# ztaylor797/APMBackend

Measured on AMD Instinct MI355X. Metric: log-lines/sec z-scored (whole node), higher is better.
Workload: dtype fp64

## Files before the change

apmbackend_amd/csrc/bindings.cpp:

```cpp
#include <pybind11/pybind11.h>
#include <pybind11/stl.h>

#include <cstring>
#include <memory>

#include "kernels/kernel_api.h"
#include "runtime/engine.h"
#include "runtime/format.h"
#include "runtime/jsutil.h"
#include "runtime/merge.h"

namespace apm {
namespace copyenc {
void encode_blob(std::string_view blob, std::string* out, int64_t* counts);
}
int apm_txcopy_lines(const char* d_text, const uint64_t* h_line_off, int64_t n, std::string& out_rows);
std::vector<double> apm_release_bench(int64_t n, int iters, uint64_t seed);
}

namespace py = pybind11;
using namespace apm;

void register_tailer(py::module_& m);
void register_synth(py::module_& m);
// ... 324 lines not shown
        py::gil_scoped_release rel;
        return c.all_reduce_host(v, max);
      }, py::arg("values"), py::arg("max") = false)
      .def("all_gather", [](Collective& c, py::bytes b) {
        std::string s = b;
        std::vector<uint8_t> v(s.begin(), s.end()), out;
        { py::gil_scoped_release rel; out = c.all_gather_host(v); }
        return py::bytes((const char*)out.data(), out.size());
      })
      .def("abort", &Collective::abort)
      .def("aborted", &Collective::aborted)
      .def_property_readonly("rank", &Collective::rank)
      .def_property_readonly("nranks", &Collective::nranks);
  py::class_<LocalGroup, std::shared_ptr<LocalGroup>>(m, "LocalCollGroup")
      .def(py::init([](int n, double timeout_ms) { return make_local_group(n, timeout_ms); }), py::arg("n"),
           py::arg("timeout_ms") = 120000.0);

  py::class_<Engine>(m, "Engine")
      .def(py::init([](const py::dict& d) { return new Engine(config_from(d)); }))
      .def("add_file", &Engine::add_file)
      .def("add_server", &Engine::add_server)
      .def("set_override", [](Engine& e, const std::string& svc, const py::dict& d) { e.set_override(svc, override_from(d)); })
      .def("clear_overrides", &Engine::clear_overrides)
      .def("refresh_series_settings", &Engine::refresh_series_settings)
      .def("stage_reconfig", [](Engine& e, const py::dict& ecfg, const py::dict& overrides, uint64_t gen) {
        const EngineConfig c = config_from(ecfg);
        ReconfigSpec r;
        r.gen = gen;
        r.n_lags = c.n_lags;
        for (int l = 0; l < MAX_LAGS; ++l) {
          r.lags[l] = c.lags[l]; r.thr[l] = c.thr[l]; r.infl[l] = c.infl[l]; r.lag_suppressed[l] = c.lag_suppressed[l];
        }
        r.alert_window = c.alert_window; r.alert_threshold = c.alert_threshold; r.both_only = c.both_only;
        r.hard_min_ms = c.hard_min_ms; r.hard_min_tpm = c.hard_min_tpm; r.hard_max_ms = c.hard_max_ms;
        r.cooldown_ms = c.cooldown_ms;
        r.interval_len = c.interval_len; r.window = c.window; r.buffer = c.buffer;
        for (auto kv : overrides) r.overrides[kv.first.cast<std::string>()] = override_from(kv.second.cast<py::dict>());
        e.stage_reconfig(r);
      }, py::arg("ecfg"), py::arg("overrides"), py::arg("gen"))
      .def("reconfig_info", [](Engine& e) {
        py::dict d;
        d["applied_gen"] = e.reconfig_applied_gen(); d["applied"] = e.reconfigs_applied();
        d["lag_set_changes"] = e.lag_set_changes();
        d["window_changes"] = e.window_changes();
        d["ring_slots"] = e.ring_slots();
        d["ring_grows"] = e.ring_grows();
        return d;
      })
      .def("lag_values", &Engine::lag_values)
      .def("cache_stats", [](Engine& e, bool drain) {
        std::vector<uint64_t> v;
        { py::gil_scoped_release rel; v = e.cache_stats(drain); }
        py::dict d;
        if (v.size() == 6) {
          d["slots"] = v[0]; d["occupied"] = v[1]; d["acct"] = v[2]; d["record"] = v[3]; d["partials"] = v[4];
          d["need"] = v[5];
        }
        return d;
      }, py::arg("drain") = true)
      .def("process_batch",
           [](Engine& e, py::buffer buf, const std::vector<std::tuple<int32_t, uint64_t, uint64_t>>& chunks,
              double now) {
             py::buffer_info bi = buf.request();
             const uint8_t* p = (const uint8_t*)bi.ptr;
             const uint64_t n = (uint64_t)(bi.size * bi.itemsize);
             auto ch = chunks_from(chunks);
             py::gil_scoped_release rel;
             e.process_batch(p, n, ch, now);
           },
           py::arg("buf"), py::arg("chunks"), py::arg("now") = -1.0)
      .def("process_batch_ptr",
           [](Engine& e, uintptr_t ptr, uint64_t n, const std::vector<std::tuple<int32_t, uint64_t, uint64_t>>& chunks,
              double now, uintptr_t next_ptr, uint64_t next_n,
              const std::vector<std::tuple<int32_t, uint64_t, uint64_t>>& next_chunks) {
             auto ch = chunks_from(chunks);
             auto nch = chunks_from(next_chunks);
             py::gil_scoped_release rel;
             e.process_batch((const uint8_t*)ptr, n, ch, now, next_ptr ? (const uint8_t*)next_ptr : nullptr, next_n,
                             next_ptr ? &nch : nullptr);
           },
           py::arg("ptr"), py::arg("n"), py::arg("chunks"), py::arg("now") = -1.0, py::arg("next_ptr") = 0,
           py::arg("next_n") = 0,
           py::arg("next_chunks") = std::vector<std::tuple<int32_t, uint64_t, uint64_t>>())
      .def("stage_batch_ptr",
           [](Engine& e, uintptr_t ptr, uint64_t n) {
             py::gil_scoped_release rel;
             e.stage_batch((const uint8_t*)ptr, n);
           },
           py::arg("ptr"), py::arg("n"))
      .def("process_tx_lines", [](Engine& e, py::bytes b, double now) {
             std::string v = b;
             py::gil_scoped_release rel;
             e.process_tx_lines(v, now);
           }, py::arg("blob"), py::arg("now") = -1.0)
      .def("take", &Engine::take, py::call_guard<py::gil_scoped_release>())
      .def("flush", &Engine::flush, py::call_guard<py::gil_scoped_release>())
      .def("dump_state", [](Engine& e, const std::string& path, const std::string& reason) {
        py::gil_scoped_release rel;
        return e.dump_state(path, reason);
      })
      .def("save_state", [](Engine& e, const std::string& path, py::bytes extra) {
             std::string x = extra;
             py::gil_scoped_release rel;
             return e.save_state(path, x);
           }, py::arg("path"), py::arg("extra") = py::bytes(""))
      .def("checkpoint_async", [](Engine& e, const std::string& prefix, py::bytes extra, bool force_base) {
             std::string x = extra;
             py::gil_scoped_release rel;
             return e.checkpoint_async(prefix, x, force_base);
           }, py::arg("prefix"), py::arg("extra") = py::bytes(""), py::arg("force_base") = false)
      .def("checkpoint_wait", &Engine::checkpoint_wait, py::call_guard<py::gil_scoped_release>())
      .def("checkpoint_info", [](Engine& e) {
        const CheckpointInfo c = e.checkpoint_info();
        py::dict d;
        d["busy"] = c.busy; d["done"] = c.done; d["skipped"] = c.skipped; d["sync_fallbacks"] = c.sync_fallbacks;
        d["chain_len"] = c.chain_len; d["last_base"] = c.last_base; d["last_stall_ms"] = c.last_stall_ms;
        d["last_write_ms"] = c.last_write_ms; d["last_bytes"] = c.last_bytes; d["stage_bytes"] = c.stage_bytes;
        d["last_deferred_bytes"] = c.last_deferred_bytes;
        d["streamed"] = c.streamed; d["streamed_live_rows"] = c.streamed_live_rows;
        d["side_rows"] = c.side_rows; d["guard_stalls"] = c.guard_stalls; d["stage_cap"] = c.stage_cap;
        d["last_ring_rows"] = c.last_ring_rows;
        return d;
      })
      .def("export_series", &Engine::export_series, py::call_guard<py::gil_scoped_release>())
      .def("import_series", &Engine::import_series, py::call_guard<py::gil_scoped_release>())
      .def("export_buckets", [](Engine& e) {
        BucketDump d;
        { py::gil_scoped_release rel; d = e.export_buckets(); }
        return py::make_tuple(d.latest, d.series, d.bucket, d.count, d.values);
      })
      .def("import_buckets", &Engine::import_buckets, py::call_guard<py::gil_scoped_release>())
      .def("export_history", [](Engine& e, int lag_idx, int32_t lo, int32_t hi) {
        std::vector<int32_t> len;
        std::vector<double> vals;
        { py::gil_scoped_release rel; e.export_history(lag_idx, lo, hi, len, vals); }
        return py::make_tuple(len, py::bytes((const char*)vals.data(), vals.size() * 8));
      })
      .def("import_history", [](Engine& e, int lag_idx, const std::vector<int32_t>& series,
                                const std::vector<int32_t>& len, py::bytes vals) {
        std::string b = vals;
        std::vector<double> v(b.size() / 8);
        std::memcpy(v.data(), b.data(), v.size() * 8);
        py::gil_scoped_release rel;
        e.import_history(lag_idx, series, len, v);
      })
      .def("export_lag_settings", &Engine::export_lag_settings)
      .def("export_pending", &Engine::export_pending, py::call_guard<py::gil_scoped_release>())
      .def("import_pending", &Engine::import_pending, py::call_guard<py::gil_scoped_release>())
      .def("export_cooldowns", &Engine::export_cooldowns)
      .def("import_cooldowns", &Engine::import_cooldowns)
      .def("export_alert_counters", &Engine::export_alert_counters)
      .def("import_alert_counters", &Engine::import_alert_counters)
      .def("cooldown_by_service", &Engine::cooldown_by_service)
      .def("set_trace", &Engine::set_trace)
      .def("take_trace", [](Engine& e) {
        std::vector<TraceEvent> t;
        { py::gil_scoped_release rel; t = e.take_trace(); }
        py::list out;
        for (auto& x : t) out.append(py::make_tuple(std::string(x.name), x.t0_ms, x.t1_ms, x.tid, x.batch));
        return out;
      })
      .def("set_server_context", &Engine::set_server_context, py::arg("server"), py::arg("ts_ms"),
           py::arg("gauges"), py::arg("host_load") = 0.0)
      .def("load_state", [](Engine& e, const std::string& path) {
             std::string x;
             { py::gil_scoped_release rel; x = e.load_state(path); }
// ... 418 lines not shown
```

apmbackend_amd/csrc/runtime/devjoin.h:

```cpp
#pragma once
#include <hip/hip_runtime.h>

#include <atomic>
#include <cstdint>
#include <deque>
#include <functional>
#include <mutex>
#include <string>
#include <unordered_map>
#include <vector>

#include "../apm_types.h"
#include "../kernels/devjoin_api.h"
#include "hipres.h"
#include "join.h"

namespace apm {

struct CopySegs;

struct DevJoinConfig {
  uint32_t max_events = 1u << 20;
  uint64_t max_batch_bytes = 64ull << 20;
  uint32_t max_chunks = 4096;
  int table_bits = 21;
  int reg_bits = 20;
  uint32_t max_raw = 1u << 20;
  uint32_t arena_cap = 1u << 20;
  uint32_t pool_blocks = 0;
  uint64_t ring_bytes = 4ull << 30;
  double record_ttl_ms = 120000, acct_ttl_ms = 120000, need_ttl_ms = 30000;
  TzTable tz{};
  int device = 0;
};

struct DevJoinBatch {
  int slot = 0;
  uint32_t n_out = 0, n_stats = 0, n_db = 0, n_dropped = 0;
  std::vector<std::pair<uint32_t, int64_t>> cands;
  std::vector<std::pair<uint32_t, int32_t>> unresolved;
  std::string text_tx, text_db;
  uint64_t ring_base = 0;
  int64_t max_bucket = INT64_MIN;
  TxRec* d_tx = nullptr;
  int32_t* d_raw = nullptr;
  int64_t* d_gid = nullptr;
};

class DeviceJoin {
 public:
  DeviceJoin(const DevJoinConfig& cfg, Dictionary* dict, const std::vector<FileInfo>* files,
             const std::vector<std::string>* servers);
  ~DeviceJoin();

  uint8_t* d_bytes(int k) { return sl_[k].d_bytes; }
  uint8_t* d_stage() {
    if (!d_stage_bytes_) {
      d_stage_bytes_ = (uint8_t*)res_.dmalloc_on(stream_, cfg_.max_batch_bytes + 256);
      HIP_OK(hipStreamSynchronize(stream_));
    }
    return d_stage_bytes_;
  }
  void swap_stage(int k) { std::swap(sl_[k].d_bytes, d_stage_bytes_); }
  Event* d_events(int k) { return sl_[k].d_events; }
  void select_host(int k, const uint32_t* d_n_ev, uint32_t max_ev, hipStream_t ps);
  void set_chunks(int k, const std::vector<int32_t>& chunk_file, const uint32_t* d_chunk_file,
                  const uint8_t* d_chunk_kind);
  void chunk_upload(int k, uint32_t max_ev, CopySegs& cs);
  void export_select(int k, CopySegs& cs);
  using ParallelFor = std::function<void(int, const std::function<void(int)>&)>;
  void run(int k, const uint8_t* host_bytes, uint32_t n_ev, uint64_t n_bytes, double now, uint64_t batch_no, bool want_tx,
           bool want_db, DevJoinBatch& out, const ParallelFor& parallel = nullptr,
           const std::function<void()>* meanwhile = nullptr);
  void prepass_ahead(int k, const uint8_t* host_bytes, const ParallelFor& parallel);
  void release_slot(int k, hipStream_t stats_stream);

  int32_t raw_server(int32_t raw) const { return raw_info_[raw].server; }
  int32_t raw_service(int32_t raw) const { return raw_info_[raw].norm_id; }
  int32_t n_raw() const { return n_raw_.load(std::memory_order_acquire); }
  int32_t* d_raw_series() { return d_raw_series_; }

  char* ring() { return d_ring_; }
  uint64_t ring_cap() const { return cfg_.ring_bytes; }
  void set_ring_low(uint64_t low);
  uint64_t ring_head() const { return ring_head_.load(std::memory_order_acquire); }
  uint64_t ring_low() const { return ring_low_.load(std::memory_order_acquire); }
  uint64_t keys_live() const { return keys_live_ + keys_since_rebuild_; }
  uint64_t need_live() const { return arena_head_ - (regions_.empty() ? arena_head_ : regions_.front().lo); }
  uint64_t ring_reserve(uint64_t bytes);
  void reset_ring(uint64_t head);

  JoinCounters counters() const;
  std::vector<uint64_t> cache_stats(double now, bool sync = true);

  void save(class BinWriter& w);
  void load(class BinReader& r);
  static constexpr int kPhases = 8;
  double phase_t[kPhases + 1] = {0};
  std::vector<std::pair<const char*, std::pair<double, double>>> spans;
  std::vector<std::pair<const char*, std::pair<double, double>>> save_spans;
  const JoinCounts& last_counts() const { return *h_counts_; }
  size_t device_bytes() const { return res_.device_bytes(); }
  size_t trim(double now);

 private:
  struct Slot {
    uint8_t* d_bytes = nullptr;
    Event* d_events = nullptr;
    uint8_t* host_flag = nullptr;
    uint32_t* d_mh_idx = nullptr;
    uint32_t* d_walk_idx = nullptr;
    AudF* d_aud = nullptr;
    SelCount* d_n_host = nullptr;
    Mapped<Event> h_host_ev;
    Mapped<uint32_t> h_host_idx;
    Mapped<SelCount> h_n_host;
    int32_t* d_chunk_next = nullptr;
    uint8_t* d_chunk_first = nullptr;
    Mapped<int32_t> h_chunk_next;
    Mapped<uint8_t> h_chunk_first;
    const uint32_t* d_chunk_file = nullptr;
    const uint8_t* d_chunk_kind = nullptr;
    uint32_t n_chunks = 0;
    std::vector<int32_t> chunk_file;
    TxRec* d_tx = nullptr;
    int32_t* d_tx_raw = nullptr;
    int64_t* d_tx_gid = nullptr;
    hipEvent_t free_ev = nullptr;
    bool used = false;
  } sl_[2];

  struct RawInfo { int32_t server; int32_t norm_id; uint64_t svc; };

  struct PrepassTask {
    int32_t file = -1;
    std::vector<uint32_t> idx;
    std::vector<HostOp> hops;
    std::string hbuf;
    uint64_t audit_errors = 0, invalid_acct = 0, pm_host = 0;
    uint32_t put(std::string_view s) { const uint32_t o = (uint32_t)hbuf.size(); hbuf.append(s.data(), s.size()); return o; }
  };
  void host_prepass(int k, const uint8_t* host_bytes, uint32_t n_host, const ParallelFor& parallel,
                    std::vector<HostOp>& hops, std::string& hbuf);
  void host_event(PrepassTask& t, const Event& e, uint32_t ev, const uint8_t* host_bytes);
  void on_app(PrepassTask& t, const Event& e, uint32_t ev, std::string_view line);
  void save_tables(class BinWriter& w);
  void aud_reserve(AudGen& g, uint32_t autr, uint32_t items, uint64_t txt);
// ... 12 lines not shown
  void grow_pool(uint64_t need_free);
  uint64_t pool_avail(bool exact);
  void ensure_tmp();

  DevJoinConfig cfg_;
  uint32_t init_table_cap_ = 0, init_arena_cap_ = 0;
  Dictionary* dict_;
  const std::vector<FileInfo>* files_;
  const std::vector<std::string>* servers_;
  hipStream_t stream_ = nullptr;
  HipRes res_;
  uint8_t* d_stage_bytes_ = nullptr;

  std::vector<HostOp> hops_;
  std::string hbuf_;
  std::vector<HostOp> hops_ahead_;
  std::string hbuf_ahead_;
  int ahead_k_ = -1;
  PinnedBuf<HostOp> h_hops_;
  PinnedBuf<uint8_t> h_hbuf_;
  HostOp* d_hops_ = nullptr;
  uint8_t* d_hbuf_ = nullptr;
  size_t d_hops_cap_ = 0, d_hbuf_cap_ = 0;
  std::vector<PrepassTask> tasks_;
  void* d_sel_tmp_ = nullptr;
  size_t sel_tmp_bytes_ = 0;
  uint64_t audit_errors_ = 0, host_pm_ = 0, host_invalid_acct_ = 0, host_events_ = 0, events_ = 0, tx_ = 0, tx_db_ = 0;

  DJArgs a_{};
  DJFormatArgs f_{};
  KeyState* d_table_ = nullptr;
  uint64_t* d_keys_ = nullptr;
  uint32_t keys_cap_ = 0;
  bool keys_stale_ = true;
  void sync_keys();
  unsigned long long* d_cstats_ = nullptr;
  unsigned long long* h_cstats_ = nullptr;
  unsigned long long cstats_last_[5] = {0, 0, 0, 0, 0};
  uint32_t cstats_cap_ = 0, cstats_last_cap_ = 0;
  hipEvent_t cstats_ev_ = nullptr;
  bool cstats_pending_ = false, cstats_have_ = false;
  KeyState* d_table_spare_ = nullptr;
  uint32_t table_cap_ = 0;
  uint64_t keys_since_rebuild_ = 0, keys_live_ = 0;
  bool live_pending_ = false;
  hipEvent_t live_ev_ = nullptr;
  uint32_t* d_rb_scratch_ = nullptr;
  size_t rb_scratch_bytes_ = 0;
  uint8_t* d_pool_ = nullptr;
  uint32_t* d_pool_ring_ = nullptr;
  uint32_t pool_n_ = 0;
  unsigned long long* h_live_ = nullptr;
  uint64_t table_grows_ = 0, arena_grows_ = 0, pool_grows_ = 0, table_rebuilds_ = 0, trims_ = 0;
  RegSlot* d_reg_ = nullptr;
  RegMiss* d_miss_ = nullptr;
  RegMiss* h_miss_ = nullptr;
  uint32_t miss_cap_ = 0;
  NeedEnt* d_arena_ = nullptr;
  uint64_t arena_head_ = 0;
  struct Region { uint64_t lo, hi; double exp; };
  std::deque<Region> regions_;
  uint64_t* d_exp_lo_ = nullptr;
  uint64_t* d_exp_hi_ = nullptr;
  Mapped<uint64_t> h_exp_;
  SoapState* d_soap_ = nullptr;
  AudGen aud_gen_[2]{};
  int aud_cur_ = 0;
  uint64_t* d_sel_val_ = nullptr;
  uint64_t* d_sel_pos_ = nullptr;
  uint64_t *d_aud_key_ = nullptr, *d_aud_key_sorted_ = nullptr;
  uint32_t *d_aud_ord_ = nullptr, *d_aud_ord_sorted_ = nullptr;
  uint32_t aud_key_cap_ = 0;
  uint32_t* d_walk_lo_ = nullptr;
  int32_t* d_file_first_ = nullptr;
  AudItem* d_aud_slots_ = nullptr;
  uint32_t aud_slots_cap_ = 0;
  static constexpr size_t kCkBounce = 32u << 20;
  char* h_ck_bounce_ = nullptr;
  uint32_t soap_cap_ = 0;
  int32_t* d_file_server_ = nullptr;
  uint64_t* d_file_skey_ = nullptr;
  uint64_t* d_file_fkey_ = nullptr;
  std::vector<uint64_t> h_file_skey_, h_file_fkey_;
  void sync_file_keys();
  size_t files_uploaded_ = 0;
  RawSvc* d_rawtab_ = nullptr;
  int32_t* d_raw_series_ = nullptr;
  int32_t* d_raw_first_ = nullptr;
  std::vector<RawInfo> raw_info_;
  std::atomic<int32_t> n_raw_{0};
  std::string names_;
  std::unordered_map<std::string, int32_t> name_off_;
  char* d_names_ = nullptr;
  size_t names_uploaded_ = 0, names_cap_ = 0;
  int32_t* d_reg_fill_ = nullptr;
  int32_t* h_reg_fill_ = nullptr;
  RawSvc* h_rawtab_ = nullptr;
  TxDev* d_out_ = nullptr;
  uint32_t out_cap_ = 0;
  uint32_t* d_lens_ = nullptr;
  uint32_t* d_offs_ = nullptr;
  int64_t* d_bucket_ = nullptr;
  int64_t* d_bmax_ = nullptr;
  uint32_t* d_cand_ = nullptr;
  int64_t* d_cand_bucket_ = nullptr;
  uint32_t* d_unres_ = nullptr;
  uint32_t* h_cand_ = nullptr;
  int64_t* h_cand_bucket_ = nullptr;
  uint32_t* h_unres_ = nullptr;
  char* d_txt_tx_ = nullptr;
  char* d_txt_db_ = nullptr;
  size_t txt_cap_ = 0;
  PinnedBuf<char> h_txt_;
  uint32_t last_tx_bytes_ = 0, last_db_bytes_ = 0, last_cands_ = 0;
  uint64_t* d_ring_pos_ = nullptr;
  uint32_t* d_slot_head_ = nullptr;
  uint32_t heads_cap_ = 0;
  uint32_t* d_big_ = nullptr;
  uint64_t write_regrows_ = 0;
  void ensure_txt(size_t bytes);
  void* d_tmp_ = nullptr;
  size_t tmp_bytes_ = 0;
  JoinCounts* d_counts_ = nullptr;
  JoinCounts* h_counts_ = nullptr;
  unsigned long long* d_live_ = nullptr;
  JOp* d_ops_ = nullptr;
  uint8_t* d_soap_code_ = nullptr;
  double* d_soap_num_ = nullptr;
  uint64_t* d_soap_hash_ = nullptr;
  uint32_t* d_chunk_ev_lo_ = nullptr;
  uint32_t* d_seg_f_ = nullptr;
  uint32_t* d_seg_in_ = nullptr;
  uint64_t* d_chain_hash_ = nullptr;
  uint32_t *d_op_slot_ = nullptr, *d_op_slot_sorted_ = nullptr, *d_op_idx_ = nullptr, *d_op_idx_sorted_ = nullptr;
  uint64_t *d_exp_key_ = nullptr, *d_exp_key_sorted_ = nullptr;
  uint32_t *d_exp_idx_ = nullptr, *d_exp_idx_sorted_ = nullptr, *d_exp_cnt_ = nullptr, *d_exp_pos_ = nullptr;
  uint32_t exp_cap_ = 0;
  uint32_t* d_out_cnt_ = nullptr;
  uint32_t* d_out_pos_ = nullptr;
  TxDev* d_stage_ = nullptr;
  DJOverflow* d_ovf_ = nullptr;
  char* d_ring_ = nullptr;
  std::mutex ring_mu_;
  std::atomic<uint64_t> ring_head_{0};
  std::atomic<uint64_t> ring_low_{0};
};

}
```

apmbackend_amd/csrc/runtime/engine.cpp:

```cpp
#include <cstdlib>
#include "engine.h"

#include <pthread.h>
#include <sched.h>

#include <cctype>
#include <fstream>

#include <rocprofiler-sdk-roctx/roctx.h>

#include <unistd.h>

#include <cerrno>
#include <cstring>

#include <algorithm>
#include <exception>
#include <chrono>
#include <cmath>
#include <cstring>
#include <queue>
#include <stdexcept>

#include "../kernels/devjoin_api.h"
// ... 663 lines not shown

void Engine::refresh_series_settings() {
  flush();
  for (int l = 0; l < MAX_LAGS; ++l) { alias_thr_[l] = cfg_.thr[l]; alias_infl_[l] = cfg_.infl[l]; }
  std::vector<int32_t> order(n_series_);
  for (int32_t i = 0; i < n_series_; ++i) order[i] = i;
  std::sort(order.begin(), order.end(), [&](int32_t a, int32_t b) { return series_[a].emit_key < series_[b].emit_key; });
  for (int32_t s : order) if (zscore_seen_[s]) apply_series_settings(s);
  upload_series_tables(0);
}

void Engine::upload_series_tables(int32_t lo) {
  const int32_t n = n_series_;
  if (lo < 0) lo = 0;
  if (n <= lo) return;
  const size_t m = (size_t)(n - lo);
  const int L = cfg_.n_lags;
  char* st = stage(m * (8 * (2 * L + 2) + 1));
  double* col = (double*)st;
  for (int l = 0; l < L; ++l) {
    double* t = col + (size_t)(2 * l) * m;
    double* f = col + (size_t)(2 * l + 1) * m;
    for (size_t i = 0; i < m; ++i) {
      t[i] = h_thr_[(size_t)(lo + i) * MAX_LAGS + l];
      f[i] = h_infl_[(size_t)(lo + i) * MAX_LAGS + l];
    }
    h2d(lag_[l].thr + lo, t, m * 8, stream_);
    h2d(lag_[l].infl + lo, f, m * 8, stream_);
  }
  double* hm = col + (size_t)(2 * L) * m;
  uint64_t* ek = (uint64_t*)(col + (size_t)(2 * L + 1) * m);
  uint8_t* sp = (uint8_t*)(col + (size_t)(2 * L + 2) * m);
  std::memcpy(hm, h_hard_max_.data() + lo, m * 8);
  std::memcpy(ek, h_emit_key_.data() + lo, m * 8);
  std::memcpy(sp, h_suppressed_.data() + lo, m);
  h2d(d_hard_max_ + lo, hm, m * 8, stream_);
  h2d(d_emit_key_ + lo, ek, m * 8, stream_);
  h2d(d_suppressed_ + lo, sp, m, stream_);
  stage_done();
  if (want(OUT_SL)) upload_slo_classes(lo);
}

void Engine::upload_slo_classes(int32_t lo) {
  const int32_t n = n_series_;
  lo = std::min(lo, slo_cls_uploaded_);
  if (lo == 0 || h_slo_cls_.size() != (size_t)n) {
    h_slo_cls_.resize((size_t)n);
    for (int32_t s = 0; s < n; ++s) h_slo_cls_[s] = slo_class_of(s);
    lo = 0;
  }
  if (n > lo) {
    const size_t mc = (size_t)(n - lo);
    int32_t* cs = (int32_t*)stage(mc * 4);
    std::memcpy(cs, h_slo_cls_.data() + lo, mc * 4);
    h2d(d_slo_cls_ + lo, cs, mc * 4, stream_);
    stage_done();
  }
  slo_cls_uploaded_ = n;
}

std::vector<uint64_t> Engine::cache_stats(bool drain) {
  if (drain) flush();
  if (dj_) {
    if (drain) HIP_OK(hipStreamSynchronize(parse_stream_));
    return dj_->cache_stats(watermark_, drain);
  }
  return {};
}

JoinCounters Engine::join_counters() const {
  if (dj_) return dj_->counters();
  JoinCounters t;
  for (auto& s : shards_) {
    const JoinCounters& c = s->counters;
    t.events += c.events; t.tx += c.tx; t.tx_db += c.tx_db; t.expired_partials += c.expired_partials;
    t.need_expired += c.need_expired; t.ejb_exit_unmatched += c.ejb_exit_unmatched;
    t.invalid_acct += c.invalid_acct; t.audit_errors += c.audit_errors; t.host_fallback += c.host_fallback;
  }
  return t;
}

void Engine::launch_parse(ParseSlot& ps, const uint8_t* host_bytes, uint64_t n_bytes, const std::vector<Chunk>& chunks_in,
                          bool speculative) {
  const double t0 = now_ms();
  if (n_bytes > cfg_.max_batch_bytes) throw std::runtime_error("batch larger than max_batch_bytes");
  if (chunks_in.size() > cfg_.max_chunks) throw std::runtime_error("too many chunks in batch");
  std::vector<size_t> order(chunks_in.size());
  for (size_t i = 0; i < order.size(); ++i) order[i] = i;
  std::stable_sort(order.begin(), order.end(), [&](size_t a, size_t b) {
    return files_[chunks_in[a].file].server < files_[chunks_in[b].file].server;
  });
  ps.chunk_file.assign(chunks_in.size(), 0);
  uint64_t off = 0;
  bool canonical = true;
  for (size_t k = 0; k < order.size(); ++k) {
    const Chunk& c = chunks_in[k];
    if (order[k] != k || c.begin != off) { canonical = false; break; }
    off = c.end;
  }
  canonical = canonical && off == n_bytes && n_bytes + 64 <= cfg_.max_batch_bytes + 256;
  ps.hb = ps.h_bytes;
  if (canonical) {
    ps.hb = host_bytes;
    for (size_t k = 0; k < order.size(); ++k) {
      const Chunk& c = chunks_in[k];
      if (c.end > c.begin && host_bytes[c.end - 1] != '\n') throw std::runtime_error("chunk must end with a newline");
      ps.h_chunk_begin[k] = (uint32_t)c.begin;
      ps.h_chunk_kind[k] = files_[c.file].kind;
      ps.h_chunk_file[k] = (uint32_t)c.file;
      ps.chunk_file[k] = c.file;
    }
  } else {
    off = 0;
    const bool in_place = host_bytes == ps.h_bytes;
    std::vector<uint8_t> tmp_copy;
    const uint8_t* src = host_bytes;
    if (in_place) {
      tmp_copy.assign(host_bytes, host_bytes + n_bytes);
      src = tmp_copy.data();
    }
    for (size_t k = 0; k < order.size(); ++k) {
      const Chunk& c = chunks_in[order[k]];
      const uint64_t len = c.end - c.begin;
      if (len > 0 && src[c.end - 1] != '\n') throw std::runtime_error("chunk must end with a newline");
      std::memcpy(ps.h_bytes + off, src + c.begin, len);
      ps.h_chunk_begin[k] = (uint32_t)off;
      ps.h_chunk_kind[k] = files_[c.file].kind;
      ps.h_chunk_file[k] = (uint32_t)c.file;
      ps.chunk_file[k] = c.file;
      off += len;
    }
    std::memset(ps.h_bytes + off, 0, 64);
  }
  const uint32_t n_chunks = (uint32_t)order.size();
  ps.h_chunk_begin[n_chunks] = (uint32_t)off;
  ps.n_bytes = off;
  ps.src = host_bytes;
  ps.src_n = n_bytes;
  metrics_.bytes += off;
  ++metrics_.batches;

  const int k = (int)(&ps - pslot_);
  bool staged = false;
  if (dev() && canonical && in_stage_src_ == host_bytes && in_stage_n_ == n_bytes && in_stage_ev_) {
    HIP_OK(hipStreamWaitEvent(parse_stream_, in_stage_ev_, 0));
    dj_->swap_stage(k);
    staged = true;
    ++metrics_.staged_batches;
  }
  in_stage_src_ = nullptr;
  in_stage_n_ = 0;
  uint8_t* dbytes = dev() ? dj_->d_bytes(k) : d_bytes_;
  Event* devents = dev() ? dj_->d_events(k) : d_events_;
  if (!staged) HIP_OK(hipMemcpyAsync(dbytes, ps.hb, off, hipMemcpyHostToDevice, parse_stream_));
  {
    CopySegs up;
    up.add(d_chunk_begin_[k], HipRes::device_alias(ps.h_chunk_begin), (size_t)(n_chunks + 1) * 4);
    up.add(d_chunk_kind_[k], HipRes::device_alias(ps.h_chunk_kind), n_chunks + 1);
    up.add(d_chunk_file_[k], HipRes::device_alias(ps.h_chunk_file), (size_t)(n_chunks + 1) * 4);
    if (dev()) {
      dj_->set_chunks(k, ps.chunk_file, d_chunk_file_[k], d_chunk_kind_[k]);
      dj_->chunk_upload(k, cfg_.max_lines, up);
    }
    apm_copy_segs(&up, parse_stream_);
  }
  if (apm_parse_batch(dbytes, off, d_chunk_begin_[k], d_chunk_kind_[k], d_chunk_file_[k], n_chunks, d_parse_ws_,
                      cfg_.max_lines, devents, d_counts_, d_counts_ + 1, d_watermark_, d_file_open_, &cfg_.tz,
                      parse_stream_) != 0)
    throw std::runtime_error("parse workspace too small");
  if (dev()) dj_->select_host(k, d_counts_, cfg_.max_lines, parse_stream_);
  {
    CopySegs ex;
    ex.add(HipRes::device_alias(ps.h_counts), d_counts_, 8);
    ex.add(HipRes::device_alias(ps.h_watermark), d_watermark_, 8);
    if (dev()) dj_->export_select(k, ex);
    apm_copy_segs(&ex, parse_stream_);
  }
  ps.spec_copied = 0;
  if (speculative && !dev() && spec_events_) {
    ps.spec_copied = std::min<uint32_t>(spec_events_, cfg_.max_lines);
    HIP_OK(hipMemcpyAsync(ps.h_events, d_events_, (size_t)ps.spec_copied * sizeof(Event), hipMemcpyDeviceToHost,
                          parse_stream_));
  }
  ps.pending = true;
  metrics_.t_parse_ms += now_ms() - t0;
}

void Engine::stage_batch(const uint8_t* host_bytes, uint64_t n_bytes) {
  if (!dev() || !host_bytes || n_bytes == 0 || n_bytes > cfg_.max_batch_bytes) return;
  const double t0 = now_ms();
  if (!in_stage_stream_) {
    HIP_OK(hipStreamCreateWithFlags(&in_stage_stream_, hipStreamNonBlocking));
    res_.adopt(in_stage_stream_);
    in_stage_ev_ = res_.new_event();
  }
  HIP_OK(hipMemcpyAsync(dj_->d_stage(), host_bytes, n_bytes, hipMemcpyHostToDevice, in_stage_stream_));
  HIP_OK(hipEventRecord(in_stage_ev_, in_stage_stream_));
  in_stage_src_ = host_bytes;
  in_stage_n_ = n_bytes;
  trace_event("stage H2D (launch)", t0, now_ms(), 0);
}

void Engine::finish_parse(ParseSlot& ps) {
  const double t0 = now_ms();
  HIP_OK(hipStreamSynchronize(parse_stream_));
  ps.n_events = ps.h_counts[0];
  ps.n_lines = ps.h_counts[1];
  if (ps.n_lines > cfg_.max_lines) throw std::runtime_error("batch has more lines than max_lines");
  metrics_.lines += ps.n_lines;
  metrics_.events += ps.n_events;
  if (!dev() && ps.n_events > ps.spec_copied) {
    const uint32_t lo = ps.spec_copied;
    HIP_OK(hipMemcpyAsync(ps.h_events + lo, d_events_ + lo, (size_t)(ps.n_events - lo) * sizeof(Event),
                          hipMemcpyDeviceToHost, parse_stream_));
    HIP_OK(hipStreamSynchronize(parse_stream_));
  }
  ps.spec_copied = 0;
  spec_events_ = ps.n_events + ps.n_events / 4 + 1024;
  ps.pending = false;
  last_slot_ = (int)(&ps - pslot_);
  metrics_.t_parse_ms += now_ms() - t0;
}

static void merge_shard_outputs(const std::vector<std::vector<TxOut>>& outs, bool multi, std::vector<TxOut>& txs) {
  txs.clear();
  const int ns = (int)outs.size();
  size_t total = 0;
  std::vector<size_t> split(ns, 0);
  for (int k = 0; k < ns; ++k) {
    auto& v = outs[k];
    total += v.size();
    size_t p = 0;
    while (p < v.size() && !(v[p].seq >> 63)) ++p;
    split[k] = p;
  }
  txs.reserve(total);
  using Item = std::pair<uint64_t, std::pair<int, size_t>>;
  std::priority_queue<Item, std::vector<Item>, std::greater<Item>> pq;
  for (int k = 0; k < ns; ++k)
    if (split[k] > 0) pq.push({outs[k][0].seq, {k, 0}});
  while (!pq.empty()) {
    auto it = pq.top();
    pq.pop();
    auto& v = outs[it.second.first];
    txs.push_back(v[it.second.second]);
    const size_t nx = it.second.second + 1;
// ... 63 lines not shown
    };
    const uint32_t nc = (uint32_t)chunk_file.size();
    uint32_t c = 0;
    while (c < nc) {
      const int32_t srv = files_[chunk_file[c]].server;
      uint32_t d = c + 1;
      while (d < nc && files_[chunk_file[d]].server == srv) ++d;
      const uint32_t lo = first_event_of_chunk(c), hi = first_event_of_chunk(d);
      if (hi > lo) shard_range[srv].push_back({lo, hi});
      c = d;
    }
  }
  shard_ms_.assign(shards_.size() * 16, 0.0);
  shard_maxb_.assign(shards_.size() * 8, INT64_MIN);
  pool_->run((int)shards_.size(), [&](int s) {
    const double ts0 = now_ms();
    JoinShard& sh = *shards_[s];
    sh.out().clear();
    sh.begin_batch(clock, batch_no_);
    for (const auto& r : shard_range[s]) sh.process(h_events + r.first, r.second - r.first, hb, chunk_file);
    if (lockstep_) {
      int64_t b = INT64_MIN;
      for (const TxOut& t : sh.out()) {
        if (t.to_db || !(t.end_ms == t.end_ms) || t.end_ms < 10000) continue;
        const int64_t tb = (int64_t)t.end_ms / 10000;
        if (tb > b) b = tb;
      }
      shard_maxb_[(size_t)s * 8] = b;
    }
    const double ts1 = now_ms();
    shard_ms_[(size_t)s * 16] = ts1 - ts0;
    trace_event("shard", ts0, ts1, 2 + s);
  }, launch_next ? &launch_next_parse : nullptr);
  const double t1b = now_ms();
  metrics_.t_join_shards_ms += t1b - t1;
  {
    double sum = 0, mx = 0;
    for (size_t s = 0; s < shards_.size(); ++s) { sum += shard_ms_[s * 16]; mx = std::max(mx, shard_ms_[s * 16]); }
    metrics_.t_shard_busy_ms += shards_.empty() ? 0 : sum / shards_.size();
    metrics_.t_shard_max_ms += mx;
  }
  std::vector<std::vector<TxOut>> outs(shards_.size());
  {
    std::lock_guard<std::mutex> g(out_pool_mu_);
    for (size_t k = 0; k < shards_.size(); ++k) {
      outs[k].swap(shards_[k]->out());
      if (!out_pool_.empty()) {
        shards_[k]->out().swap(out_pool_.back());
        out_pool_.pop_back();
      }
    }
  }
  bool multi = false;
  for (auto& r : shard_range) multi |= r.size() > 1;
  const double t2 = now_ms();
  metrics_.t_join_ms += t2 - t1;
  metrics_.t_merge_ms += t2 - t1b;
  roctxRangePop();
  trace_event("join", t1, t1b, 0);
  trace_event("handoff", t1b, t2, 0);

  int sync_slot = -1;
  if (lockstep_) {
    int64_t bmax = INT64_MIN;
    for (size_t k = 0; k < shards_.size(); ++k) bmax = std::max(bmax, shard_maxb_[k * 8]);
    sync_slot = lockstep_collect(bmax);
  } else {
    watermark_ = batch_watermark(ps);
  }

  const double tp0 = now_ms();
  post_stats(std::move(outs), multi, t0, sync_slot);
  const double tp1 = now_ms();
  trace_event("post", tp0, tp1, 0);
  if (coll_) fleet_exchange_upto(fleet_posted_ - 1);
  trace_event("fleet.exchange", tp1, now_ms(), 0);
  metrics_.t_total_ms += now_ms() - t0;
  ++batch_no_;
}

void Engine::process_batch_dev_tail(ParseSlot& ps, double t0, double now_override, const uint8_t* next_bytes,
                                    uint64_t next_n, const std::vector<Chunk>* next_chunks) {
  const int k = (int)(&ps - pslot_);
  if (next_bytes && next_chunks) {
    launch_parse(pslot_[k ^ 1], next_bytes, next_n, *next_chunks, true);
    prefetched_ = true;
  }
  cur_slot_ = k ^ 1;
  last_n_events_ = ps.n_events;
  const double t1 = now_ms();
  roctxRangePop();
  roctxRangePushA("apm.join");
  trace_event("parse", t0, t1, 0);
  const double clock = now_override >= 0 ? now_override : watermark_;
  if (lockstep_) lockstep_issue(batch_watermark(ps));
  DevJoinBatch b;
  const DeviceJoin::ParallelFor par = [this](int n, const std::function<void(int)>& fn) { pool_->run(n, fn); };
  const std::function<void()> ahead = [this, k, par]() {
    if (!ahead_lane_) ahead_lane_.reset(new TaskLane());
    ahead_task_ = ahead_lane_->post([this, k, par]() {
      ParseSlot& nx = pslot_[k ^ 1];
      const double ta = now_ms();
      finish_parse(nx);
      dj_->prepass_ahead(k ^ 1, nx.hb, par);
      trace_event("next parse+prepass", ta, now_ms(), 3);
    });
  };
  const bool do_ahead = prefetched_;
  const std::function<void()> meanwhile = [this, &ahead, do_ahead]() {
    if (do_ahead) ahead();
    if (coll_ && fleet_due_ > fleet_rounds_) {
      const double tf = now_ms();
      fleet_exchange_upto(fleet_due_);
      trace_event("fleet.exchange", tf, now_ms(), 0);
    }
  };
  dj_->run(k, ps.hb, ps.n_events, ps.n_bytes, clock, batch_no_, want(OUT_TRANSACTIONS), want(OUT_AUDIT_DB), b, par,
           &meanwhile);
  const double t2 = now_ms();
  metrics_.t_join_ms += t2 - t1;
  metrics_.t_join_shards_ms += t2 - t1;
  metrics_.t_shard_max_ms += t2 - t1;
  metrics_.t_shard_busy_ms += t2 - t1;
  roctxRangePop();
  trace_event("join (GPU)", t1, t2, 0);
  if (trace_on_) {
    static const char* names[DeviceJoin::kPhases] = {"dj.prepass", "dj.upload", "dj.launch", "dj.syncA",
                                                     "dj.register", "dj.plan", "dj.write+syncC", "dj.tail"};
    for (int i = 0; i < DeviceJoin::kPhases; ++i) trace_event(names[i], dj_->phase_t[i], dj_->phase_t[i + 1], 2);
    for (const auto& sp : dj_->spans) trace_event(sp.first, sp.second.first, sp.second.second, 2);
  }
  const int sync_slot = lockstep_ ? lockstep_collect(b.max_bucket) : -1;
  if (!lockstep_) watermark_ = batch_watermark(ps);
  const double tp0 = now_ms();
  post_stats_dev(std::move(b), t0, sync_slot);
  const double tp1 = now_ms();
  trace_event("post", tp0, tp1, 0);
  if (coll_) fleet_due_ = fleet_posted_ - 1;
  metrics_.t_total_ms += now_ms() - t0;
  ++batch_no_;
}

void Engine::process_tx_lines(const std::string& blob, double now) {
  if (dev()) throw std::runtime_error("process_tx_lines needs gpu.joinOnDevice = false");
  const double t0 = now_ms();
  std::vector<std::vector<TxOut>> outs(shards_.size());
  uint64_t line = 0;
  size_t i = 0;
  while (i < blob.size()) {
    size_t j = blob.find('\n', i);
    if (j == std::string::npos) j = blob.size();
    const std::string_view ln(blob.data() + i, j - i);
    i = j + 1;
    if (ln.size() < 3 || ln.compare(0, 3, "tx|") != 0) continue;
    std::string_view f[9];
    int nf = 0;
    size_t a = 0;
    while (nf < 9) {
      const size_t b = ln.find('|', a);
      f[nf++] = ln.substr(a, b == std::string_view::npos ? std::string_view::npos : b - a);
      if (b == std::string_view::npos) break;
      a = b + 1;
    }
    if (nf < 8) { ++metrics_.tx_dropped; continue; }
    const std::string srv(f[1]);
    const auto known = server_ids_.find(srv);
    const int32_t sid = known != server_ids_.end() ? known->second : add_server(srv);
    if ((size_t)sid >= outs.size()) outs.resize(shards_.size());
    const int32_t svc = dict_.service_id(f[2]);
    std::string& arena = shards_[sid]->text();
    TxOut t{};
    t.seq = (1ULL << 63) | (line++ << 12);
    t.server = sid;
    t.service = svc;
    t.raw_svc = svc;
    t.end_ms = js::parse_int(f[6]);
    t.elapsed = js::parse_int(f[7]);
    t.line_off = (uint32_t)arena.size();
    t.line_len = (uint32_t)ln.size();
    t.to_db = false;
    t.toplevel = nf > 8 && f[8] == "Y";
    arena.append(ln.data(), ln.size());
    arena += '\n';
    outs[sid].push_back(t);
  }
  if (now >= 0 && now > watermark_) watermark_ = now;
  outs.resize(shards_.size());
  metrics_.lines += line;
  post_stats(std::move(outs), true, t0, -1);
  metrics_.t_total_ms += now_ms() - t0;
  ++batch_no_;
}

void Engine::trace_event(const char* name, double t0, double t1, int tid) {
  if (!trace_on_) return;
  std::lock_guard<std::mutex> g(trace_mu_);
  if (trace_.size() < 1000000) trace_.push_back(TraceEvent{name, t0, t1, tid, batch_no_});
}

std::vector<TraceEvent> Engine::take_trace() {
  flush();
  std::lock_guard<std::mutex> g(trace_mu_);
  std::vector<TraceEvent> r;
  r.swap(trace_);
  return r;
}
// ... 2641 lines not shown
```

apmbackend_amd/csrc/runtime/engine.h:

```cpp
#pragma once
#include <hip/hip_runtime.h>

#include "binio.h"

#include <array>
#include <atomic>
#include <condition_variable>
#include <cstdint>
#include <deque>
#include <functional>
#include <map>
#include <memory>
#include <mutex>
#include <string>
#include <thread>
#include <tuple>
#include <unordered_map>
#include <vector>

#include "../apm_types.h"
#include "../kernels/kernel_api.h"
#include "collective.h"
#include "devjoin.h"
#include "hipres.h"
// ... 576 lines not shown
    if ((size_t)server >= ser_tab_.size()) ser_tab_.resize((size_t)server + 1);
    auto& row = ser_tab_[server];
    if ((size_t)service >= row.size()) row.resize(std::max<size_t>((size_t)service + 1, row.size() * 2), -1);
    row[service] = s;
  }
  std::vector<SeriesInfo> series_;
  int32_t n_series_ = 0;
  std::vector<int32_t> server_rank_;
  std::vector<int32_t> server_next_service_;
  int32_t next_server_rank_ = 0;
  std::map<std::string, ServiceOverride> overrides_;
  double alias_thr_[MAX_LAGS], alias_infl_[MAX_LAGS];
  std::vector<double> h_thr_, h_infl_, h_hard_max_;
  std::vector<uint8_t> h_suppressed_;
  std::vector<uint64_t> h_emit_key_;
  std::vector<int32_t> zscore_seen_;
  std::vector<uint8_t> h_active_;
  std::vector<int32_t> unseen_;

  std::unique_ptr<DeviceJoin> dj_;
  const DevJoinBatch* cur_dj_ = nullptr;
  uint64_t ring_low_pending_ = UINT64_MAX;
  unsigned long long* d_ring_min_ = nullptr;
  Mapped<unsigned long long> h_ring_min_;
  int64_t* d_rel_n_ = nullptr;
  Mapped<int64_t> h_rel_n_;
  uint32_t* d_rel_lens_ = nullptr;
  uint32_t* d_rel_offs_ = nullptr;
  uint32_t* d_rel_fb_ = nullptr;
  Mapped<uint32_t> h_rel_total_;
  char* d_rel_text_[2] = {nullptr, nullptr};
  size_t rel_text_cap_[2] = {0, 0};
  PinnedBuf<char> h_rel_text_[REL_RING];
  int rel_ring_k_ = 0;
  PinnedBuf<uint32_t> h_rel_offs_[2];
  hipStream_t out_stream_ = nullptr;
  std::vector<int32_t> h_raw_series_;
  static constexpr int kStage = 32;
  PinnedBuf<char> h_stage_[kStage];
  size_t stage_max_ = 0;
  hipEvent_t stage_ev_[kStage] = {};
  int stage_k_ = 0;
  void h2d(void* d, const void* h_pinned, size_t n, hipStream_t s);
  void d2h(void* h_pinned, const void* d, size_t n, hipStream_t s);
  char* stage(size_t bytes);
  void stage_done();
  int32_t* d_pairs_ = nullptr;
  size_t pairs_bytes_ = 0;
  int32_t* pinned_pairs(size_t n_ints);
  void pinned_pairs_done() { stage_done(); }
  size_t max_name_len_ = 0;
  int32_t* d_unseen_idx_ = nullptr;
  uint8_t* d_unseen_flag_ = nullptr;
  uint8_t* h_unseen_flag_ = nullptr;
  unsigned long long* d_unmapped_ = nullptr;
  bool dev() const { return dj_ != nullptr; }

  uint8_t* d_bytes_ = nullptr;
  struct ParseSlot {
    uint8_t* h_bytes = nullptr;
    uint32_t* h_chunk_begin = nullptr;
    uint8_t* h_chunk_kind = nullptr;
    uint32_t* h_chunk_file = nullptr;
    Event* h_events = nullptr;
    uint32_t* h_counts = nullptr;
    unsigned long long* h_watermark = nullptr;
    const uint8_t* hb = nullptr;
    const uint8_t* src = nullptr;
    uint64_t src_n = 0, n_bytes = 0;
    std::vector<int32_t> chunk_file;
    uint32_t n_events = 0, n_lines = 0;
    uint32_t spec_copied = 0;
    bool pending = false;
  } pslot_[2];
  uint32_t spec_events_ = 0;
  int cur_slot_ = 0, last_slot_ = 0;
  bool prefetched_ = false;
  const uint8_t* in_stage_src_ = nullptr;
  uint64_t in_stage_n_ = 0;
  hipStream_t in_stage_stream_ = nullptr;
  hipEvent_t in_stage_ev_ = nullptr;
  void launch_parse(ParseSlot& ps, const uint8_t* host_bytes, uint64_t n_bytes, const std::vector<Chunk>& chunks,
                    bool speculative = false);
  void process_batch_dev_tail(ParseSlot& ps, double t0, double now_override, const uint8_t* next_bytes,
                              uint64_t next_n, const std::vector<Chunk>* next_chunks);
  void finish_parse(ParseSlot& ps);
  double batch_watermark(const ParseSlot& ps) const;
  uint32_t* d_chunk_begin_[2] = {nullptr, nullptr};
  uint8_t* d_chunk_kind_[2] = {nullptr, nullptr};
  uint32_t* d_chunk_file_[2] = {nullptr, nullptr};
  void* d_parse_ws_ = nullptr;
  Event* d_events_ = nullptr;
  uint32_t* d_counts_ = nullptr;
  unsigned long long* d_watermark_ = nullptr;
  uint8_t* d_file_open_ = nullptr;
  TzTable* d_tz_unused_ = nullptr;

  int32_t* d_counts_cells_ = nullptr;
  int32_t* d_cells_ = nullptr;
  int32_t* d_spill_n_ = nullptr;
  int32_t* d_spill_series_ = nullptr;
  int32_t* d_spill_val_ = nullptr;
  int32_t* d_spill_series_alt_ = nullptr;
  int32_t* d_spill_val_alt_ = nullptr;
  void* d_spill_tmp_ = nullptr;
  size_t spill_tmp_bytes_ = 0;
  Mapped<int32_t> h_spill_snap_;
  uint64_t spill_added_ = 0;
  std::vector<uint64_t> spill_clear_at_;
  struct SpillMark { hipEvent_t ev = nullptr; uint64_t added = 0; bool live = false; };
  static constexpr int kSpillMarks = 4;
  SpillMark spill_mark_[kSpillMarks];
  int spill_mark_k_ = 0;
  void spill_reserve(uint32_t n);
  void spill_marked();
  void spill_resync();
  void grow_spill(int32_t cap);
  void spill_sort();
  unsigned long long* d_spill_drop_ = nullptr;
  uint8_t* d_active_ = nullptr;
  int32_t nslot_ = NSLOT_MIN;
  std::vector<int64_t> slot_bucket_;
  uint64_t ring_grows_ = 0;
  int32_t* d_win_slots_ = nullptr;
  void alloc_ring(int32_t nslot);
  void grow_ring(int32_t nslot);
  int64_t latest_ = 0;
  int64_t rollover_idx_ = 0;
  WinStat* d_win_ = nullptr;
  int32_t* d_big_list_ = nullptr;
  int32_t* d_big_n_ = nullptr;
  int32_t* d_nan_until_ = nullptr;
  int32_t* d_ord_list_ = nullptr;
  int32_t* d_ord_n_ = nullptr;
  int32_t* d_nan_list_ = nullptr;
  int32_t* d_nan_n_ = nullptr;
  int32_t* d_js_scratch_ = nullptr;
  static constexpr int32_t kJsCap = 1 << 18;
  StatsState stats_state() const;
  void grow_tx_capacity(uint32_t need, uint32_t keep);
  int64_t ord_cap_ = 0;

  struct CkJob {
    struct Lag { int32_t n_cols = 0; std::vector<int32_t> heads; size_t off = 0; };
    bool streamed = false;
    bool base = false;
    int64_t seq = 0;
    std::string prefix, name, path, extra;
    MemBlob blob;
    std::vector<Lag> lags;
    std::function<void()> pre_commit;
    std::vector<std::array<size_t, 3>> holes;
    std::vector<std::pair<size_t, int32_t>> patches;
  };
  static constexpr int kMaxChain = 16;
  enum : uint8_t { CKR_NONE = 0, CKR_LIVE, CKR_READING, CKR_STAGED, CKR_SIDE, CKR_DONE };
  struct CkStream {
    bool on = false;
    std::vector<std::vector<uint8_t>> state;
    std::vector<std::vector<size_t>> off;
    size_t side_used = 0, side_cap = 0;
    bool side_sync = false;
    int32_t n_cols = 0;
    uint64_t live_rows = 0, side_rows = 0, stalls = 0;
  } cks_;
  std::mutex cks_mu_;
// ... 320 lines not shown
```

Baseline: 320.8 million.

## Defer next-batch parse kernel launch into the join's meanwhile window

Launching the next batch's parse is split into two steps: input staging (host-to-device copy, chunk setup, file-key sync) and kernel launch. The copy is still issued before the current join, but the parse kernels are now launched inside the meanwhile callback that runs while the join is in progress. The aim is to stop next-batch parse kernels from competing with the early join work, while still overlapping them with the join. In exchange it adds exception rollback of the half-started batch's metrics, subtracts the launch time from the join metrics, and exposes a prefetch_pending binding.

```diff
diff --git a/apmbackend_amd/csrc/bindings.cpp b/apmbackend_amd/csrc/bindings.cpp
--- a/apmbackend_amd/csrc/bindings.cpp
+++ b/apmbackend_amd/csrc/bindings.cpp
@@ -430,6 +430,7 @@
            py::arg("ptr"), py::arg("n"), py::arg("chunks"), py::arg("now") = -1.0, py::arg("next_ptr") = 0,
            py::arg("next_n") = 0,
            py::arg("next_chunks") = std::vector<std::tuple<int32_t, uint64_t, uint64_t>>())
+      .def("prefetch_pending", &Engine::prefetch_pending)
       .def("stage_batch_ptr",
            [](Engine& e, uintptr_t ptr, uint64_t n) {
              py::gil_scoped_release rel;
diff --git a/apmbackend_amd/csrc/runtime/devjoin.h b/apmbackend_amd/csrc/runtime/devjoin.h
--- a/apmbackend_amd/csrc/runtime/devjoin.h
+++ b/apmbackend_amd/csrc/runtime/devjoin.h
@@ -63,6 +63,7 @@
   }
   void swap_stage(int k) { std::swap(sl_[k].d_bytes, d_stage_bytes_); }
   Event* d_events(int k) { return sl_[k].d_events; }
+  void sync_file_keys();
   void select_host(int k, const uint32_t* d_n_ev, uint32_t max_ev, hipStream_t ps);
   void set_chunks(int k, const std::vector<int32_t>& chunk_file, const uint32_t* d_chunk_file,
                   const uint8_t* d_chunk_kind);
@@ -241,7 +242,6 @@
   uint64_t* d_file_skey_ = nullptr;
   uint64_t* d_file_fkey_ = nullptr;
   std::vector<uint64_t> h_file_skey_, h_file_fkey_;
-  void sync_file_keys();
   size_t files_uploaded_ = 0;
   RawSvc* d_rawtab_ = nullptr;
   int32_t* d_raw_series_ = nullptr;
diff --git a/apmbackend_amd/csrc/runtime/engine.cpp b/apmbackend_amd/csrc/runtime/engine.cpp
--- a/apmbackend_amd/csrc/runtime/engine.cpp
+++ b/apmbackend_amd/csrc/runtime/engine.cpp
@@ -769,6 +769,12 @@
 
 void Engine::launch_parse(ParseSlot& ps, const uint8_t* host_bytes, uint64_t n_bytes, const std::vector<Chunk>& chunks_in,
                           bool speculative) {
+  launch_parse_input(ps, host_bytes, n_bytes, chunks_in);
+  launch_parse_kernels(ps, speculative);
+}
+
+void Engine::launch_parse_input(ParseSlot& ps, const uint8_t* host_bytes, uint64_t n_bytes,
+                                const std::vector<Chunk>& chunks_in) {
   const double t0 = now_ms();
   if (n_bytes > cfg_.max_batch_bytes) throw std::runtime_error("batch larger than max_batch_bytes");
   if (chunks_in.size() > cfg_.max_chunks) throw std::runtime_error("too many chunks in batch");
@@ -828,6 +834,7 @@
   ++metrics_.batches;
 
   const int k = (int)(&ps - pslot_);
+  if (dev()) dj_->sync_file_keys();
   bool staged = false;
   if (dev() && canonical && in_stage_src_ == host_bytes && in_stage_n_ == n_bytes && in_stage_ev_) {
     HIP_OK(hipStreamWaitEvent(parse_stream_, in_stage_ev_, 0));
@@ -838,17 +845,24 @@
   in_stage_src_ = nullptr;
   in_stage_n_ = 0;
   uint8_t* dbytes = dev() ? dj_->d_bytes(k) : d_bytes_;
+  if (dev()) dj_->set_chunks(k, ps.chunk_file, d_chunk_file_[k], d_chunk_kind_[k]);
+  if (!staged) HIP_OK(hipMemcpyAsync(dbytes, ps.hb, off, hipMemcpyHostToDevice, parse_stream_));
+  metrics_.t_parse_ms += now_ms() - t0;
+}
+
+void Engine::launch_parse_kernels(ParseSlot& ps, bool speculative) {
+  const double t0 = now_ms();
+  const int k = (int)(&ps - pslot_);
+  const uint64_t off = ps.n_bytes;
+  const uint32_t n_chunks = (uint32_t)ps.chunk_file.size();
+  uint8_t* dbytes = dev() ? dj_->d_bytes(k) : d_bytes_;
   Event* devents = dev() ? dj_->d_events(k) : d_events_;
-  if (!staged) HIP_OK(hipMemcpyAsync(dbytes, ps.hb, off, hipMemcpyHostToDevice, parse_stream_));
   {
     CopySegs up;
     up.add(d_chunk_begin_[k], HipRes::device_alias(ps.h_chunk_begin), (size_t)(n_chunks + 1) * 4);
     up.add(d_chunk_kind_[k], HipRes::device_alias(ps.h_chunk_kind), n_chunks + 1);
     up.add(d_chunk_file_[k], HipRes::device_alias(ps.h_chunk_file), (size_t)(n_chunks + 1) * 4);
-    if (dev()) {
-      dj_->set_chunks(k, ps.chunk_file, d_chunk_file_[k], d_chunk_kind_[k]);
-      dj_->chunk_upload(k, cfg_.max_lines, up);
-    }
+    if (dev()) dj_->chunk_upload(k, cfg_.max_lines, up);
     apm_copy_segs(&up, parse_stream_);
   }
   if (apm_parse_batch(dbytes, off, d_chunk_begin_[k], d_chunk_kind_[k], d_chunk_file_[k], n_chunks, d_parse_ws_,
@@ -1078,10 +1092,13 @@
 void Engine::process_batch_dev_tail(ParseSlot& ps, double t0, double now_override, const uint8_t* next_bytes,
                                     uint64_t next_n, const std::vector<Chunk>* next_chunks) {
   const int k = (int)(&ps - pslot_);
+  ParseSlot& nx = pslot_[k ^ 1];
+  bool half = false;
   if (next_bytes && next_chunks) {
-    launch_parse(pslot_[k ^ 1], next_bytes, next_n, *next_chunks, true);
-    prefetched_ = true;
-  }
+    launch_parse_input(nx, next_bytes, next_n, *next_chunks);
+    half = true;
+  }
+  double t_next_kernels = 0;
   cur_slot_ = k ^ 1;
   last_n_events_ = ps.n_events;
   const double t1 = now_ms();
@@ -1102,22 +1119,40 @@
       trace_event("next parse+prepass", ta, now_ms(), 3);
     });
   };
-  const bool do_ahead = prefetched_;
-  const std::function<void()> meanwhile = [this, &ahead, do_ahead]() {
-    if (do_ahead) ahead();
+  const std::function<void()> meanwhile = [this, &ahead, &nx, &half, &t_next_kernels]() {
+    if (half) {
+      const double tk = now_ms();
+      launch_parse_kernels(nx, true);
+      half = false;
+      prefetched_ = true;
+      t_next_kernels = now_ms() - tk;
+      trace_event("next parse (launch)", tk, tk + t_next_kernels, 0);
+      ahead();
+    }
     if (coll_ && fleet_due_ > fleet_rounds_) {
       const double tf = now_ms();
       fleet_exchange_upto(fleet_due_);
       trace_event("fleet.exchange", tf, now_ms(), 0);
     }
   };
-  dj_->run(k, ps.hb, ps.n_events, ps.n_bytes, clock, batch_no_, want(OUT_TRANSACTIONS), want(OUT_AUDIT_DB), b, par,
-           &meanwhile);
+  try {
+    dj_->run(k, ps.hb, ps.n_events, ps.n_bytes, clock, batch_no_, want(OUT_TRANSACTIONS), want(OUT_AUDIT_DB), b, par,
+             &meanwhile);
+  } catch (...) {
+    if (half) {
+      metrics_.bytes -= nx.n_bytes;
+      --metrics_.batches;
+      nx.src = nullptr;
+      nx.src_n = 0;
+    }
+    throw;
+  }
   const double t2 = now_ms();
-  metrics_.t_join_ms += t2 - t1;
-  metrics_.t_join_shards_ms += t2 - t1;
-  metrics_.t_shard_max_ms += t2 - t1;
-  metrics_.t_shard_busy_ms += t2 - t1;
+  const double t_join = t2 - t1 - t_next_kernels;
+  metrics_.t_join_ms += t_join;
+  metrics_.t_join_shards_ms += t_join;
+  metrics_.t_shard_max_ms += t_join;
+  metrics_.t_shard_busy_ms += t_join;
   roctxRangePop();
   trace_event("join (GPU)", t1, t2, 0);
   if (trace_on_) {
diff --git a/apmbackend_amd/csrc/runtime/engine.h b/apmbackend_amd/csrc/runtime/engine.h
--- a/apmbackend_amd/csrc/runtime/engine.h
+++ b/apmbackend_amd/csrc/runtime/engine.h
@@ -682,6 +682,8 @@
   hipEvent_t in_stage_ev_ = nullptr;
   void launch_parse(ParseSlot& ps, const uint8_t* host_bytes, uint64_t n_bytes, const std::vector<Chunk>& chunks,
                     bool speculative = false);
+  void launch_parse_input(ParseSlot& ps, const uint8_t* host_bytes, uint64_t n_bytes, const std::vector<Chunk>& chunks);
+  void launch_parse_kernels(ParseSlot& ps, bool speculative);
   void process_batch_dev_tail(ParseSlot& ps, double t0, double now_override, const uint8_t* next_bytes,
                               uint64_t next_n, const std::vector<Chunk>* next_chunks);
   void finish_parse(ParseSlot& ps);
```

Result: no change. 324.2 million (median of 3 runs) (+1.1%).
